# ComputationalRobotics/cuADMM

Measured on AMD Instinct MI355X. Metric: ADMM iters/sec, 10k x 32-blk synthetic per GPU (+ PSD-proj TFLOP/s in roofline), higher is better.
Workload: dtype f64

## Files before the change

### cuadmm_amd/_lib.py

```python
import ctypes as C
import os

from . import build as _build

_HERE = os.path.dirname(os.path.abspath(__file__))
LIB_PATH = os.path.join(_HERE, "lib", "libcuadmm_amd.so")

c_int_p = C.POINTER(C.c_int)
c_double_p = C.POINTER(C.c_double)
ALLREDUCE_FN = C.CFUNCTYPE(C.c_int, C.c_void_p, C.c_void_p, C.c_size_t, C.c_void_p)


class ProblemView(C.Structure):
    _fields_ = [("vec_len", C.c_int), ("con_num", C.c_int), ("mat_num", C.c_int),
                ("At_nnz", C.c_int), ("b_nnz", C.c_int), ("C_nnz", C.c_int),
                ("At_csc_col_ptrs", c_int_p), ("At_csc_row_ids", c_int_p), ("At_csc_vals", c_double_p),
                ("b_indices", c_int_p), ("b_vals", c_double_p), ("C_indices", c_int_p), ("C_vals", c_double_p),
                ("blk_vals", c_int_p)]


PROTOTYPES = {
    "cuadmm_last_error": (C.c_char_p, []),
    "cuadmm_version": (C.c_char_p, []),
    "cuadmm_device_count": (C.c_int, []),
# ... 27 lines not shown
    "cuadmm_get_shard": (C.c_int, [C.c_void_p, C.POINTER(C.c_int64), C.POINTER(C.c_int64), c_int_p, c_int_p]),
    "cuadmm_aat_factor_arrays": (C.c_int, [C.c_void_p] + [C.POINTER(C.c_void_p)] * 4),
    "cuadmm_aat_forest": (C.c_int, [C.c_void_p, c_int_p, c_int_p, C.POINTER(C.c_void_p), C.POINTER(C.c_void_p)]),
    "cuadmm_mex_call": (C.c_int, [C.c_int, C.c_int, C.c_double,
                                   C.c_size_t, C.c_size_t, C.c_void_p, C.c_void_p, C.c_void_p,
                                   C.c_size_t, C.c_void_p, C.c_void_p, C.c_void_p,
                                   C.c_size_t, C.c_void_p, C.c_void_p, C.c_void_p,
                                   C.c_size_t, C.c_void_p,
                                   C.c_size_t, C.c_void_p, C.c_size_t, C.c_void_p, C.c_size_t, C.c_void_p,
                                   C.c_double, C.c_int, C.c_void_p, C.POINTER(C.c_void_p)]),
    "cuadmm_mex_result_dims": (C.c_int, [C.c_void_p, c_int_p, c_int_p, c_int_p, C.POINTER(C.c_double)]),
    "cuadmm_mex_result_XyS": (C.c_int, [C.c_void_p, C.c_void_p, C.c_void_p, C.c_void_p]),
    "cuadmm_mex_result_info": (C.c_int, [C.c_void_p, C.c_int, C.c_void_p]),
    "cuadmm_mex_result_free": (None, [C.c_void_p]),
    "cuadmm_get_psd_steps": (C.c_int, [C.c_void_p, C.c_void_p, C.c_int]),
    "cuadmm_sign_sched_simulate_hint": (C.c_int, [C.c_void_p, C.c_int, C.c_int, C.c_int, c_double_p, c_int_p]),
    "cuadmm_sign_sched_simulate": (C.c_int, [C.c_void_p, C.c_int, C.c_int, c_double_p]),
    "cuadmm_op_psd_project_ex": (C.c_int, [C.c_void_p, C.c_void_p, C.c_void_p, C.c_int, C.c_int, C.c_void_p, C.c_void_p]),
    "cuadmm_op_psd_project_steps": (C.c_int, [C.c_void_p, C.c_void_p, C.c_void_p, C.c_int, C.c_void_p, C.c_void_p]),
    "cuadmm_get_info_iter_num": (C.c_int, [C.c_void_p]),
    "cuadmm_get_info_array": (C.c_int, [C.c_void_p, C.c_int, C.c_void_p, C.c_int]),
    "cuadmm_get_total_time": (C.c_double, [C.c_void_p]),
    "cuadmm_get_state": (C.c_int, [C.c_void_p, C.c_void_p]),
    "cuadmm_get_profile": (C.c_int, [C.c_void_p, C.c_void_p]),
    "cuadmm_reset_profile": (C.c_int, [C.c_void_p]),
    "cuadmm_get_counters": (C.c_int, [C.c_void_p, C.c_void_p]),
    "cuadmm_get_group_info": (C.c_int, [C.c_void_p, C.c_void_p]),
    "cuadmm_get_tail_info": (C.c_int, [C.c_void_p, C.c_void_p]),
    "cuadmm_update_A": (C.c_int, [C.c_void_p, C.c_void_p, C.c_int, C.c_int, C.c_double]),
    "cuadmm_get_update_info": (C.c_int, [C.c_void_p, C.c_void_p]),
# ... 118 lines not shown
```

### cuadmm_amd/csrc/engine.hip

```cpp
#include <hip/hip_runtime.h>

#include <algorithm>
#include <chrono>
#include <cmath>
#include <cstdlib>
#include <cstring>
#include <dlfcn.h>
#include <iostream>
#include <numeric>

#include "device_util.h"
#include "psd_plan.h"
#include "tail_solve.h"
#include "lead_solve.h"
#include "vec_kernels.h"
#include "duo_group.h"
#include "accel.h"
#include "infeas.h"

using namespace cuadmm;

namespace {

double wall_s() { return std::chrono::duration<double>(std::chrono::steady_clock::now().time_since_epoch()).count(); }
// ... 501 lines not shown
      fz.outX = mode == 0 ? out_w : nullptr;
      fz.outS = out_w + m + 2;
    }
    if (closed.active) {
      fz.rec = closed.rec.p; fz.cl_out = closed.cl_out.p; fz.y_out = y_d.p;
      fz.iter0 = (int)(closed.iters_done & 0x3fffffff);
      closed.iters_done += iters > 1 ? iters : 1;
      fz.partials2 = closed.partials2.p;
      fz.isig = 1 / sig; fz.bscale = bscale;
      if (closed.out_dirty) {
        if ((rc = launch_closed_gather_out(closed.rec.p, plan.fused_blocks(), out_d.p, out_d.p + (size_t)m + 2, closed.cl_out.p, st))) return rc;
        closed.out_dirty = false;
      }
    }
    if (iters > 1) {
      fz.iters = iters; fz.pstride = bt.pstride; fz.partials = bt.p1.p; fz.partials2 = bt.p2.p;
      prof_begin(K_PSD);
      rc = plan.project(Xb.p, Xproj.p, st, &fz);
      prof_end(K_PSD, 68.0 * (double)L * iters);
      if (rc) return rc;
      prof_begin(K_POST);
      double* dst = (!dev_scalars && bt.h_dev) ? bt.h_dev : bt.scal_d.p;
      rc = launch_reduce_quads_batch(bt.p1.p, bt.p2.p, plan.fused_blocks(), bt.pstride, iters, dst, st);
      prof_end(K_POST, 0.0);
      if (rc) return rc;
      if (dev_scalars && (rc = comm_allreduce(bt.scal_d.p, 4 * (size_t)iters))) return rc;
      if (dst == bt.scal_d.p) CUADMM_HIP_TRY(hipMemcpyAsync(bt.h.p, bt.scal_d.p, sizeof(double) * 4 * (size_t)iters, hipMemcpyDeviceToHost, st));
      bt.launches++; bt.iters += iters;
      return CUADMM_OK;
    }
    prof_begin(K_PSD);
// ... 2112 lines not shown

int cuadmm_get_profile(const cuadmm_solver* s, double out[3 * CUADMM_NUM_KCLASS]) {
  if (!s || !out) { set_error("get_profile: null"); return CUADMM_ERR_INVALID; }
  for (int k = 0; k < K_NUM; ++k) { out[3 * k] = s->prof_count[k]; out[3 * k + 1] = s->prof_ms[k]; out[3 * k + 2] = s->prof_bytes[k]; }
  return CUADMM_OK;
}
int cuadmm_get_psd_steps(cuadmm_solver* s, int* out, int cap) {
  if (!s || !out) { set_error("get_psd_steps: null"); return CUADMM_ERR_INVALID; }
  if (!s->steps_d.p && s->psd_steps && s->initialised && s->blk_local.empty()) return 0;
  if (!s->steps_d.p) { set_error("get_psd_steps: set option psd_steps=1 before init"); return CUADMM_ERR_INVALID; }
  const int n = (int)std::min<size_t>(s->steps_d.n, (size_t)std::max(cap, 0));
  CUADMM_HIP_TRY(hipStreamSynchronize(s->st));
  { int rc2 = staged_d2h(out, s->steps_d.p, sizeof(int) * (size_t)n, s->st); if (rc2) return rc2; }
  return n;
}
int cuadmm_get_counters(const cuadmm_solver* s, double o[8]) {
  if (!s || !o) { set_error("get_counters: null"); return CUADMM_ERR_INVALID; }
  o[0] = (double)s->bt.launches; o[1] = (double)s->bt.iters; o[2] = (double)s->bt.rollbacks; o[3] = (double)cuadmm_host_pool_threads();
  o[4] = s->fuse ? 1 : 0; o[5] = s->closed.active ? 1 : 0; o[6] = s->dev_solve ? (s->lead.tops ? 3 : 1) : (s->lead.hybrid ? 2 : 0); o[7] = (double)s->tail.k;
  return CUADMM_OK;
}
int cuadmm_get_accel_info(const cuadmm_solver* s, double o[8]) {
  if (!s || !o) { set_error("get_accel_info: null"); return CUADMM_ERR_INVALID; }
  o[0] = (double)s->aa.mem; o[1] = (double)s->aa.taken; o[2] = (double)s->aa.accepted; o[3] = (double)s->aa.rejected; o[4] = (double)s->aa.restarts;
  o[5] = (double)s->aa.cols; o[6] = s->profile ? s->aa.ms : 0.0; o[7] = (double)(s->aa.ring_dF.n + s->aa.ring_dG.n) * sizeof(double);
  return CUADMM_OK;
}
int cuadmm_accel_solve_ls(const double* gram, const double* rhs, int cols, double reg, double* gamma_out) {
  return accel_solve_ls(gram, rhs, cols, reg, gamma_out);
}
// ... 408 lines not shown
```

### cuadmm_amd/csrc/psd_fuse.h

```cpp
#pragma once

namespace cuadmm {

struct SignFuse {
  const int* rp; const int* ci; const double* av;
  const double* y; const double* C;
  double* X; double* Rd1; double* S;
  double* partials;
  double sig, inv_sig, tau_sig;
  int mode;
  const struct LcDesc* lc; const int* lc_row; const int* lc_nzptr; const int* lc_e; const double* lc_v;
  double* outX; double* outS;
  double* y_out;
  double* partials2;
  double isig, bscale;
  int iters;
  long long pstride;
  const struct ClosedRec* rec;
  double* cl_out;
  int iter0;
  int full;
};
struct LcDesc { int x, y, z, w; };
constexpr int kFuseRowsMax = 64;
constexpr int kClosedMaxRows = 8;

struct alignas(64) ClosedRec {
  int nk, nnz, nrounds, maxlen;
  unsigned char nzp[16];
  int rows[kClosedMaxRows];
  unsigned nzt[kFuseRowsMax];
  unsigned char rk[kFuseRowsMax];
// ... 13 lines not shown
```

### cuadmm_amd/csrc/psd_kernels.hip

```cpp
#include <hip/hip_runtime.h>

#include <algorithm>
#include <cstdio>
#include <cstdlib>
#include <string>
#include <vector>

#include "device_util.h"
#include "eig_large.h"
#include "psd_device.h"
#include "psd_plan.h"
#include "psd_small_reg.h"
#include "psd_sign_lds.h"
#include "psd_sign_wave.h"
#include "psd_sign_closed.h"

namespace cuadmm {

struct PsdArgs {
  const double* in;
  double* out;
  double* Wout;
  int* info;
  const int* ids;
// ... 102 lines not shown
  if (m >= count) return;
  const PsdDesc d = a.desc[first + m];
  const int id = d.id;
  const long long off = d.off;
  psd_sign_wave_body<NT, FUSED, !(NT == 1 && OCC == 8)>(a.in + off, a.out + off, d.n, a.info, swt_smem, a.steps ? a.steps + id : nullptr,
                                a.hint ? a.hint + id : nullptr, a.dbg ? a.dbg + 10 * (long long)m : nullptr, fz, off, d.slot, id);
}

template <int NT, int OCC, bool FULL>
__global__ __launch_bounds__(64) __attribute__((amdgpu_waves_per_eu(OCC, OCC))) void psd_sign_closed_kernel(ClosedArgs a) {
  extern __shared__ double swt_smem[];
  const int m = (int)blockIdx.x;
  if (m >= a.count) return;
  const PsdDesc d = a.desc[a.first + m];
  SwcKArg ka = (SwcKArg)__builtin_amdgcn_kernarg_segment_ptr();
  psd_sign_closed_body<NT, false, FULL>(a, d.n, swt_smem, a.steps ? a.steps + d.id : nullptr, a.hint ? a.hint + d.id : nullptr, nullptr, d.off, d.slot, 0, d.pad[0], 0, ka);
}

__host__ __device__ constexpr int closed_cu_ctl_ints(int nb_max) { return (nb_max + 2 + 3) & ~3; }
static_assert(sizeof(PsdDesc) == 32, "the LDS descriptor cache copies a descriptor as two 16-byte words");

template <int NT, int WAVES, int OCC, bool FULL, bool DBG>
__global__ __launch_bounds__(64 * WAVES) __attribute__((amdgpu_waves_per_eu(OCC, OCC))) void psd_sign_closed_cu_kernel(ClosedArgs a) {
  extern __shared__ double swt_smem[];
  constexpr int TILE = SignWaveT<NT>::NP * SignWaveT<NT>::LD;
  int* ctl = reinterpret_cast<int*>(swt_smem + (size_t)WAVES * TILE);
  const int g = (int)blockIdx.x, G = (int)gridDim.x;
  const int nb = (a.count - g + G - 1) / G;
  for (int i = (int)threadIdx.x; i < nb + 1; i += 64 * WAVES) ctl[i] = 0;
  sl_v4i32* dcache = reinterpret_cast<sl_v4i32*>(ctl + closed_cu_ctl_ints((a.count + G - 1) / G));
  if (a.dcache)
    for (int i = (int)threadIdx.x; i < nb; i += 64 * WAVES) {
      const sl_v4i32* src = reinterpret_cast<const sl_v4i32*>(a.desc + a.first + g + i * G);
      dcache[2 * i] = src[0];
      dcache[2 * i + 1] = src[1];
    }
  __syncthreads();
  const int ntask = nb * a.iters;
  const long long clk0 = (DBG && a.dbg) ? (long long)__builtin_readcyclecounter() : 0, rt0 = (DBG && a.dbg) ? (long long)__builtin_amdgcn_s_memrealtime() : 0;
  using KArgC = __attribute__((address_space(4))) const char;
  KArgC* ka = (KArgC*)__builtin_amdgcn_kernarg_segment_ptr();
#pragma unroll 1
  for (;;) {
    const long long tk0 = (DBG && a.dbg) ? (long long)__builtin_readcyclecounter() : 0;
    int t = 0;
    if (lane_id() == 0) t = atomicAdd(&ctl[0], 1);
    t = __builtin_amdgcn_readfirstlane(t);
    if (t >= ntask) break;
    const int it = t / nb, j = t - it * nb;
    if (it > 0) {
      while (__hip_atomic_load(ctl + 1 + j, __ATOMIC_RELAXED, __HIP_MEMORY_SCOPE_WORKGROUP) < it) __builtin_amdgcn_s_sleep(8);
    }
    __builtin_amdgcn_fence(__ATOMIC_ACQUIRE, "workgroup");
    const long long tk1 = (DBG && a.dbg) ? (long long)__builtin_readcyclecounter() : 0;
#if defined(__HIP_DEVICE_COMPILE__)
    asm volatile("" : "+s"(ka));
    const ClosedArgs al = *reinterpret_cast<__attribute__((address_space(4))) const ClosedArgs*>(ka);
#else
    const ClosedArgs al = a;
    (void)ka;
#endif
    PsdDesc d;
    if (al.dcache) {
      const sl_v4i32 q0 = dcache[2 * j], q1 = dcache[2 * j + 1];
      d.off = (long long)(((unsigned long long)(unsigned)__builtin_amdgcn_readfirstlane(q0[1]) << 32) | (unsigned)__builtin_amdgcn_readfirstlane(q0[0]));
      d.n = __builtin_amdgcn_readfirstlane(q0[2]); d.id = __builtin_amdgcn_readfirstlane(q0[3]); d.slot = __builtin_amdgcn_readfirstlane(q1[0]);
      d.pad[0] = __builtin_amdgcn_readfirstlane(q1[1]);
    } else {
      d = al.desc[al.first + g + j * G];
    }
    int toff = ((int)threadIdx.x >> 6) * TILE;
#if defined(__HIP_DEVICE_COMPILE__)
    asm volatile("" : "+v"(toff));
#endif
    double* tile = swt_smem + toff;
    const long long tk2 = (DBG && al.dbg) ? (long long)__builtin_readcyclecounter() : 0;
    psd_sign_closed_body<NT, true, FULL, DBG>(al, d.n, tile, al.steps ? al.steps + d.id : nullptr, al.hint ? al.hint + d.id : nullptr,
                             (DBG && al.dbg) ? al.dbg + 16 * (long long)(g + j * G) : nullptr, d.off, d.slot, (long long)it * al.pstride, d.pad[0], it, ka);
    const long long tk3 = (DBG && al.dbg) ? (long long)__builtin_readcyclecounter() : 0;
    __builtin_amdgcn_fence(__ATOMIC_RELEASE, "workgroup");
    if (lane_id() == 0) __hip_atomic_store(ctl + 1 + j, it + 1, __ATOMIC_RELAXED, __HIP_MEMORY_SCOPE_WORKGROUP);
    if (DBG && al.dbg && lane_id() == 0) {
      long long* q = al.dbg + 16 * (long long)(g + j * G);
      q[10] = tk1 - tk0; q[11] = tk2 - tk1; q[12] = tk3 - tk2; q[13] = (long long)__builtin_readcyclecounter() - tk3;
    }
  }
  if (DBG && a.dbg && threadIdx.x == 0) {
    long long* q = a.dbg + 16 * (long long)g;
    q[14] = (long long)__builtin_readcyclecounter() - clk0; q[15] = (long long)__builtin_amdgcn_s_memrealtime() - rt0;
  }
}

template <void (*KERN)(ClosedArgs)>
static int launch_closed_cu(dim3 grid, dim3 block, size_t lds, hipStream_t st, const ClosedArgs& ca) {
  static LdsCapOnce once;
  CUADMM_HIP_TRY(once(reinterpret_cast<const void*>(KERN)));
  hipLaunchKernelGGL(KERN, grid, block, lds, st, ca);
  return CUADMM_OK;
}

template <int NT, int OCC>
static int launch_sign_wave(const PsdArgs& a, int first, int count, hipStream_t st, const SignFuse* fz = nullptr) {
  if (count <= 0) return CUADMM_OK;
  if (fz && fz->rec) {
    ClosedArgs ca{};
    ca.desc = a.desc; ca.steps = a.steps; ca.hint = a.hint; ca.fail = a.info; ca.dbg = a.dbg;
    ca.X = fz->X; ca.S = fz->S; ca.Rd1 = fz->Rd1; ca.C = fz->C; ca.rec = fz->rec; ca.cl_out = fz->cl_out; ca.y_out = fz->y_out;
    ca.outS = fz->outS; ca.outX = fz->outX; ca.partials = fz->partials; ca.partials2 = fz->partials2;
    ca.sig = fz->sig; ca.inv_sig = fz->inv_sig; ca.tau_sig = fz->tau_sig; ca.isig = fz->isig; ca.bscale = fz->bscale;
    ca.iter0 = fz->iter0;
    ca.pstride = fz->pstride; ca.mode = fz->mode; ca.iters = fz->iters > 1 ? fz->iters : 1; ca.first = first; ca.count = count;
    if (fz->iters > 1) {
      constexpr int WAVES = 4 * OCC > 16 ? 16 : 4 * OCC, WG_PER_CU = 4 * OCC / WAVES;
      static int n_cu_of[64] = {0};
      int dev = 0;
      CUADMM_HIP_TRY(hipGetDevice(&dev));
      int& n_cu = n_cu_of[dev & 63];
      if (n_cu == 0) {
        int v = 0;
        CUADMM_HIP_TRY(hipDeviceGetAttribute(&v, hipDeviceAttributeMultiprocessorCount, dev));
        n_cu = v > 0 ? v : 256;
      }
      const int grid = std::min(count, n_cu * WG_PER_CU);
      const size_t nb_max = ((size_t)count + grid - 1) / grid;
      size_t lds = WAVES * SignWaveT<NT>::LDS_BYTES + sizeof(int) * (size_t)closed_cu_ctl_ints((int)nb_max);
      ca.dcache = lds + sizeof(PsdDesc) * nb_max <= kMaxLdsBytes;
      if (ca.dcache) lds += sizeof(PsdDesc) * nb_max;
      if (lds > kMaxLdsBytes) { set_error("psd: %d blocks per workgroup do not fit the batched launch", (int)nb_max); return CUADMM_ERR_INVALID; }
      constexpr bool HAS_DBG = NT == 2 && OCC == 4;
      const dim3 gr(grid), bl(64 * WAVES);
      int rc;
      if (HAS_DBG && ca.dbg) rc = fz->full ? launch_closed_cu<psd_sign_closed_cu_kernel<NT, WAVES, OCC, true, HAS_DBG>>(gr, bl, lds, st, ca)
                                           : launch_closed_cu<psd_sign_closed_cu_kernel<NT, WAVES, OCC, false, HAS_DBG>>(gr, bl, lds, st, ca);
      else rc = fz->full ? launch_closed_cu<psd_sign_closed_cu_kernel<NT, WAVES, OCC, true, false>>(gr, bl, lds, st, ca)
                         : launch_closed_cu<psd_sign_closed_cu_kernel<NT, WAVES, OCC, false, false>>(gr, bl, lds, st, ca);
      if (rc) return rc;
    } else if (fz->full) {
      hipLaunchKernelGGL((psd_sign_closed_kernel<NT, OCC, true>), dim3(count), dim3(64), SignWaveT<NT>::LDS_BYTES, st, ca);
// ... 497 lines not shown
```

### cuadmm_amd/csrc/psd_options.h

```cpp
#pragma once
#include <cstdlib>
#include <cstring>
#include <string>

namespace cuadmm {

struct PsdOptions {
  int n16_sign = 1;
  int n32_sign = 1;
  int mid = 0;
  int wave4_min = 1024;
  int w32_occ = 4;
  int cu_occ = 4;
  int lds_triple = 1;
  int sign_min = 65;
  int overlap = 1;
  int lg_tile = 0;
  int lg_pad32 = 1;
  int lg_decide = 0;
  int lg_merge = 1;
  int lg_fuse = 1;
  int lg_cluster_wgs = 224;
  int lg_cluster = 1;
  int sign_maxsteps = 0;
  int sign_sync = 1;
  int sign_ws_mb = 8192;
  int debug = 0;

  static PsdOptions from_env() {
    PsdOptions o;
    static const struct { const char* env; const char* key; } tab[] = {
        {"CUADMM_PSD_DEBUG", "psd_debug"},           {"CUADMM_PSD_WAVE4_MIN", "psd_wave4_min"}, {"CUADMM_PSD_SIGN_MIN", "psd_sign_min"},
        {"CUADMM_PSD_W32_OCC", "psd_w32_occ"},       {"CUADMM_PSD_CU_OCC", "psd_cu_occ"},       {"CUADMM_PSD_OVERLAP", "psd_overlap"},
        {"CUADMM_PSD_N16", "psd_n16"},               {"CUADMM_PSD_N32", "psd_n32"},             {"CUADMM_PSD_MID", "psd_mid"},
        {"CUADMM_PSD_LG_CLUSTER", "psd_lg_cluster"}, {"CUADMM_PSD_LDS_TRIPLE", "psd_lds_triple"}, {"CUADMM_PSD_LG_MERGE", "psd_lg_merge"},
        {"CUADMM_PSD_LG_FUSE", "psd_lg_fuse"},       {"CUADMM_PSD_LG_CLUSTER_WGS", "psd_lg_cluster_wgs"}};
    for (const auto& t : tab)
      if (const char* e = getenv(t.env)) {
        int v;
        if (!strcmp(e, "eig")) v = strcmp(t.key, "psd_mid") ? 0 : 1;
        else if (!strcmp(e, "lds")) v = 2;
        else v = atoi(e);
        o.set(t.key, v);
      }
    return o;
  }
  bool set(const std::string& k, double value) {
    const int v = (int)value;
    if (k == "psd_n16") n16_sign = v;
    else if (k == "psd_n32") n32_sign = v;
    else if (k == "psd_mid") mid = v;
    else if (k == "psd_wave4_min") wave4_min = v;
    else if (k == "psd_w32_occ") w32_occ = v == 3 ? 3 : 4;
    else if (k == "psd_cu_occ") cu_occ = v == 3 ? 3 : 4;
    else if (k == "psd_lds_triple") lds_triple = v;
    else if (k == "psd_sign_min") sign_min = v < 65 ? 65 : v;
    else if (k == "psd_overlap") overlap = v;
    else if (k == "psd_lg_tile") lg_tile = v;
    else if (k == "psd_lg_pad32") lg_pad32 = v;
    else if (k == "psd_lg_decide") lg_decide = v;
    else if (k == "psd_lg_cluster") lg_cluster = v;
    else if (k == "psd_lg_merge") lg_merge = v;
    else if (k == "psd_lg_fuse") lg_fuse = v;
    else if (k == "psd_lg_cluster_wgs") lg_cluster_wgs = v < 8 ? 8 : (v > 960 ? 960 : v);
    else if (k == "psd_sign_maxsteps") sign_maxsteps = v;
    else if (k == "psd_sign_sync") sign_sync = v;
    else if (k == "psd_sign_ws_mb") sign_ws_mb = v < 1 ? 1 : v;
    else if (k == "psd_debug") debug = v < 0 ? 0 : v;
    else return false;
// ... 6 lines not shown
```

### cuadmm_amd/csrc/psd_sign_closed.h

```cpp
#pragma once
#include <hip/hip_runtime.h>

#include "psd_sign_wave.h"

namespace cuadmm {

template <int LD>
__device__ __forceinline__ int swc_sym(int row, int col) { return row <= col ? row * LD + col : col * LD + row; }
template <int LD, int NP>
__device__ __forceinline__ int swc_low(int r, int c) { return r == c ? r * LD + NP : c * LD + r; }

template <int NT>
__device__ __forceinline__ void swc_frags(const double* __restrict__ M, int r16, int kk, double (&f)[4 * NT][NT]) {
  constexpr int LD = SignWaveT<NT>::LD;
#pragma unroll
  for (int s = 0; s < 4 * NT; ++s)
#pragma unroll
    for (int x = 0; x < NT; ++x) {
      const int b = s / 4, row = 4 * s + kk, col = 16 * x + r16;
      if (x > b) f[s][x] = M[row * LD + col];
      else if (x < b) f[s][x] = M[col * LD + row];
      else f[s][x] = M[swc_sym<LD>(row, col)];
    }
}
// ... 78 lines not shown
template <int NT> __device__ const SwcTab<NT> g_swc_tab = SwcTab<NT>();

struct ClosedArgs {
  const PsdDesc* desc;
  int* steps; int* hint; int* fail;
  long long* dbg;
  double* X; double* S; double* Rd1; const double* C;
  const ClosedRec* rec;
  double* cl_out; double* y_out; double* outS; double* outX;
  double* partials; double* partials2;
  double sig, inv_sig, tau_sig, isig, bscale;
  long long pstride;
  int mode, iters, first, count;
  int iter0;
  int dcache;
};

using SwcKArg = __attribute__((address_space(4))) const char*;
template <bool RELOAD>
__device__ __forceinline__ ClosedArgs swc_args(const ClosedArgs& fz, SwcKArg& ka) {
#if defined(__HIP_DEVICE_COMPILE__)
  if (RELOAD) {
    asm volatile("" : "+s"(ka));
    return *reinterpret_cast<__attribute__((address_space(4))) const ClosedArgs*>(ka);
  }
#endif
  return fz;
}

#define CUADMM_SWC_STAMP(k) \
  if (dbg) { asm volatile("s_waitcnt vmcnt(0) lgkmcnt(0)" ::: "memory"); if (lane == 0) dbg[k] = (long long)__builtin_readcyclecounter() - c0; }

template <int NT, bool TASK_LOOP = false, bool FULL = false, bool DBG = false>
__device__ __forceinline__ void psd_sign_closed_body(const ClosedArgs& fz, int n_arg, double* S, int* steps_out, int* hint, long long* dbg_arg,
                                                     long long off, int slot, long long poff, int hdr, int it_local, SwcKArg ka) {
  long long* const dbg = DBG ? dbg_arg : nullptr;
  using Cfg = SignWaveT<NT>;
  constexpr int LD = Cfg::LD, NP = Cfg::NP, U = Cfg::U, NSLOT = Cfg::NSLOT;
  constexpr int NB = (NSLOT + U - 1) / U;
  const int n = FULL ? NP : n_arg;
  int lane_p = lane_id();
#if defined(__HIP_DEVICE_COMPILE__)
  if (TASK_LOOP) asm volatile("" : "+v"(lane_p));
  __builtin_assume(lane_p >= 0 && lane_p < 64);
#endif
  const int lane = lane_p;
  const int r16 = lane & 15, kk = lane >> 4;
  const int len = n * (n + 1) / 2;
  const int ksteps = FULL ? 4 * NT : ((n + 3) >> 2);
  const long long c0 = dbg ? (long long)__builtin_readcyclecounter() : 0;
  const bool upd = fz.mode == 0;
  const ClosedRec* __restrict__ rec = fz.rec + slot;
  const unsigned* __restrict__ tabl = g_swc_tab<NT>.v + lane;
  const double* __restrict__ Xl = fz.X + off + lane;
  const double* __restrict__ Cl = fz.C + off + lane;
  auto at = [&](unsigned byte_off) -> double& { return *reinterpret_cast<double*>(reinterpret_cast<char*>(S) + byte_off); };

  const int nk = closed_hdr_nk(hdr), nnz = closed_hdr_nnz(hdr), nrounds = closed_hdr_nrounds(hdr);
  const int l8 = lane & 7;
  const bool mine = lane < nk;
  const double nzv = rec->v[lane];
  const unsigned nzt = rec->nzt[lane];
  const int nzrk = rec->rk[lane];
  const int row = rec->rows[l8];
  const double dk = rec->D[l8], bk = rec->b[l8];
  const double ax_old = fz.cl_out[16 * (long long)slot + l8], as_old = fz.cl_out[16 * (long long)slot + 8 + l8];
  double lrow[kClosedMaxRows], lcol[kClosedMaxRows];
#pragma unroll
  for (int q = 0; q < kClosedMaxRows; ++q) {
    lrow[q] = rec->L[l8 * kClosedMaxRows + q];
    lcol[q] = rec->L[q * kClosedMaxRows + l8];
  }
  unsigned tb[U];
  double xv[U], cv[U];
#pragma unroll
  for (int u = 0; u < U; ++u) { tb[u] = tabl[64 * u]; xv[u] = Xl[64 * u]; cv[u] = Cl[64 * u]; }
  {
    sl_v2f64* S2 = reinterpret_cast<sl_v2f64*>(S);
    double zero = 0.0;
#if defined(__HIP_DEVICE_COMPILE__)
    if (TASK_LOOP) asm volatile("" : "+v"(zero));
#endif
#pragma unroll 1
    for (int i = lane; i < NP * LD / 2; i += 64) S2[i] = sl_v2f64{zero, zero};
    wave_fence();
  }
  double yk = 0.0;
  if (nk > 0) {
    const double rp = __dadd_rn(-ax_old, bk);
    double x = mine ? __dadd_rn(-as_old, __dmul_rn(fz.isig, rp)) : 0.0;
#pragma unroll
// ... 39 lines not shown
      if (ok_) {
        at(lo) = r1;
        if (!upd) fz.Rd1[off + e_] = r1;
        ss += xb * xb;
        at(up) = (tb[u] & 1u) ? xb : xb * kSqrt2Inv;
      }
    }
  }
  CUADMM_SWC_STAMP(6);
  const double nrm = sqrt(wave_sum(ss));
  const double scale = nrm > 0.0 ? 1.0 / nrm : (nrm == 0.0 ? 0.0 : nrm);
  wave_fence();
  double f[4 * NT][NT];
  SignSchedPlain sched;
  if (hint) {
    int h = __builtin_amdgcn_readfirstlane(*hint);
    if (h > 1 && (((unsigned)fz.iter0 + (unsigned)it_local + (unsigned)slot) & 15u) == 15u) --h;
    if (h > 0) sched.lift0 = h;
  }
  bool last = false;
  const long long c1 = dbg ? (long long)__builtin_readcyclecounter() : 0;
  while (!last) {
    swc_frags<NT>(S, r16, kk, f);
    if (sched.steps == 0) {
#pragma unroll
      for (int s = 0; s < 4 * NT; ++s)
#pragma unroll
        for (int x = 0; x < NT; ++x) f[s][x] *= scale;
    }
    wave_fence();
    sl_v4f64 y[NT][NT];
// ... 48 lines not shown
    }
    double alpha, beta;
    sched.coefs(mu, alpha, beta);
#pragma unroll
    for (int i = 0; i < NT; ++i)
#pragma unroll
      for (int j = i; j < NT; ++j)
#pragma unroll
        for (int r = 0; r < 4; ++r) z[i][j][r] = fma(alpha, z[i][j][r], beta * f[4 * i + r][j]);
    wave_fence();
    swc_store_upper<NT>(S, r16, kk, z);
    wave_fence();
  }
  if (steps_out && lane == 0) *steps_out = sched.steps;
  if (hint && lane == 0) *hint = sched.lifts;
  const long long c2 = dbg ? (long long)__builtin_readcyclecounter() : 0;
  int lane_e = lane;
#if defined(__HIP_DEVICE_COMPILE__)
  asm volatile("" : "+v"(lane_e));
#endif
  const unsigned* __restrict__ tabl_e = g_swc_tab<NT>.v + lane_e;
  const ClosedArgs fe = swc_args<true>(fz, ka);
  const ClosedRec* __restrict__ rec_e = fe.rec + slot;
  const double* __restrict__ Xl_e = fe.X + off + lane_e;
  const double* __restrict__ Cl_e = fe.C + off + lane_e;
  const int l8e = lane_e & 7;
  const bool mine_e = lane_e < nk;
#pragma unroll
  for (int u = 0; u < U; ++u) { tb[u] = tabl_e[64 * u]; xv[u] = Xl_e[64 * u]; }
  swc_frags<NT>(S, r16, kk, f);
// ... 77 lines not shown
#pragma unroll
    for (int u = 0; u < U; ++u) {
      const int e_ = base + 64 * u + lane_e;
      const bool ok_ = (FULL && base + 64 * u + 63 < Cfg::MAXLEN) || e_ < len;
      const unsigned up = tb[u] & 0xfff8u, lo = tb[u] >> 16;
      const double pm = at(up), r1 = at(lo);
      bad |= ok_ && !(fabs(pm) <= 1.7976931348623157e308);
      const double xp = (tb[u] & 1u) ? pm : pm * kSqrt2;
      const double x = xv[u];
      const double xdiff = xp - x;
      const double sv = fw.inv_sig * xdiff - r1;
      double xn = x;
      double rd = 0.0;
      if (upd) { rd = r1 + sv; xn = x + fw.tau_sig * rd; }
      if (ok_) {
        Sg[base + 64 * u] = sv;
        if (upd) {
          Xg[base + 64 * u] = xn;
          s_rd += rd * rd;
          s_cx += cv[u] * xn;
        }
        at(up) = sv - cv[u];
        at(lo) = xn;
      }
      if ((u % 3) == 2) swc_sched_split();
    }
  }
  CUADMM_SWC_STAMP(9);
  {
    wave_fence();
    const double ps = nzv_e * at(nzt_e & 0xfff8u);
    const double px = nzv_e * at(nzt_e >> 16);
    const int maxlen = closed_hdr_maxlen(hdr);
    double as = 0.0, ax = 0.0;
    for (int t = 0; t < maxlen; ++t) {
      const int src = (kb + t) & 63;
      const double vs = __shfl(ps, src, 64), vx = __shfl(px, src, 64);
      if (mine_e && kb + t < ke) { as += vs; ax += vx; }
    }
    if (mine_e) {
      fw.outS[row_e] = as;
      fw.cl_out[16 * (long long)slot + 8 + lane_e] = as;
      if (upd) { fw.outX[row_e] = ax; fw.cl_out[16 * (long long)slot + lane_e] = ax; }
    }
    if (upd) {
      const double ro = nrmA_e * (bk_e - ax) * fw.bscale;
      double pr = mine_e ? ro * ro : 0.0;
      pr = wave_sum(pr);
      const double pby = pby_sum;
      s_rd = wave_sum(s_rd);
      s_cx = wave_sum(s_cx);
      if (lane_e == 0) {
        fw.partials2[poff + 2 * (long long)slot] = pr; fw.partials2[poff + 2 * (long long)slot + 1] = pby;
        fw.partials[poff + 2 * (long long)slot] = s_rd; fw.partials[poff + 2 * (long long)slot + 1] = s_cx;
      }
    }
  }
  if (bad && fw.fail) atomicAdd(fw.fail, 1);
  if (dbg && lane == 0) {
// ... 8 lines not shown
```

### cuadmm_amd/solver.py

```python
import ctypes as C

import numpy as np

from . import _lib
from ._lib import check

_INFO = {"pobj": 0, "dobj": 1, "errRp": 2, "errRd": 3, "relgap": 4, "sig": 5, "bscale": 6, "Cscale": 7}


def _i32(a):
    return np.ascontiguousarray(a, dtype=np.int32)


def _f64(a):
    return np.ascontiguousarray(a, dtype=np.float64)


def _p(a):
    return None if a is None else a.ctypes.data_as(C.c_void_p)


class Problem:

    def __init__(self, vec_len, con_num, blk_vals, At_csc_col_ptrs, At_csc_row_ids, At_csc_vals,
# ... 257 lines not shown
        return dict(zip(keys, o.tolist()))

    def profile(self):
        o = np.zeros(24)
        check(self._lib.cuadmm_get_profile(self._h, _p(o)))
        names = ["aty_xb", "psd_project", "post_proj", "spmv_A", "copies", "host", "allreduce", "tail_solve"]
        return {n: dict(launches=o[3 * i], ms=o[3 * i + 1], bytes_per_launch=o[3 * i + 2]) for i, n in enumerate(names)}

    def psd_steps(self):
        b, e, kb, ke = self.shard()
        out = np.zeros(max(ke - kb, 1), np.int32)
        n = self._lib.cuadmm_get_psd_steps(self._h, _p(out), out.size)
        check(min(n, 0))
        return out[:n]

    def reset_profile(self):
        check(self._lib.cuadmm_reset_profile(self._h))
```

### include/cuadmm_amd.h

```cpp
#ifndef CUADMM_AMD_H
#define CUADMM_AMD_H

#include <stddef.h>
#include <stdint.h>

#ifdef __cplusplus
extern "C" {
#endif

#define CUADMM_OK 0
#define CUADMM_ERR_INVALID (-1)
#define CUADMM_ERR_NO_DEVICE (-2)
#define CUADMM_ERR_IO (-3)
#define CUADMM_ERR_FACTOR (-4)
#define CUADMM_ERR_EIG (-5)
#define CUADMM_ERR_COMM (-6)
#define CUADMM_ERR_ALLOC (-7)
#define CUADMM_ERR_INTERNAL (-8)

const char* cuadmm_last_error(void);
const char* cuadmm_version(void);
int cuadmm_device_count(void);

typedef struct cuadmm_solver cuadmm_solver;
// ... 54 lines not shown
#define CUADMM_INFO_ERRRP 2
#define CUADMM_INFO_ERRRD 3
#define CUADMM_INFO_RELGAP 4
#define CUADMM_INFO_SIG 5
#define CUADMM_INFO_BSCALE 6
#define CUADMM_INFO_CSCALE 7
int cuadmm_get_info_iter_num(const cuadmm_solver* s);
int cuadmm_get_info_array(const cuadmm_solver* s, int which, double* out, int cap);
double cuadmm_get_total_time(const cuadmm_solver* s);
int cuadmm_get_state(const cuadmm_solver* s, double out12[12]);

#define CUADMM_NUM_KCLASS 8
int cuadmm_get_profile(const cuadmm_solver* s, double out[3 * CUADMM_NUM_KCLASS]);
int cuadmm_reset_profile(cuadmm_solver* s);
int cuadmm_get_psd_steps(cuadmm_solver* s, int* out, int cap);
int cuadmm_get_counters(const cuadmm_solver* s, double out8[8]);
int cuadmm_get_tail_info(const cuadmm_solver* s, double out[6]);
int cuadmm_get_accel_info(const cuadmm_solver* s, double out8[8]);
int cuadmm_accel_solve_ls(const double* gram, const double* rhs, int cols, double reg, double* gamma_out);
int cuadmm_get_status(const cuadmm_solver* s, double out8[8]);
int cuadmm_get_certificate(cuadmm_solver* s, double* y_out, double* X_out);
int cuadmm_infeas_decide(const double stats[8], double tol, int* verdict, double* radius);
int cuadmm_get_group_info(const cuadmm_solver* s, double out4[4]);

typedef struct cuadmm_problem cuadmm_problem;
typedef struct {
  int vec_len, con_num, mat_num;
  int At_nnz, b_nnz, C_nnz;
  const int* At_csc_col_ptrs;
  const int* At_csc_row_ids;
// ... 128 lines not shown
```

Measured before the change: 5058.

## Run consecutive ADMM iterations per block in closed PSD task loop with register carry

The persistent closed-form PSD kernel now processes a run of consecutive iterations (default 2) for the same block within one task, rather than one iteration per task. Per-block state (X, C, table entries, record values, hint, ax/as) is carried in registers between iterations, which avoids global reloads and skips the intermediate S stores that later iterations overwrite. The aim is to cut global memory traffic and atomic task-scheduling overhead. In exchange, the pipeline across blocks gets coarser, which can worsen load balance, and register pressure rises. An optional workgroup cap and a debug accessor for the PSD hints are also added.

```diff
diff --git a/cuadmm_amd/_lib.py b/cuadmm_amd/_lib.py
--- a/cuadmm_amd/_lib.py
+++ b/cuadmm_amd/_lib.py
@@ -65,6 +65,7 @@
     "cuadmm_mex_result_info": (C.c_int, [C.c_void_p, C.c_int, C.c_void_p]),
     "cuadmm_mex_result_free": (None, [C.c_void_p]),
     "cuadmm_get_psd_steps": (C.c_int, [C.c_void_p, C.c_void_p, C.c_int]),
+    "cuadmm_get_psd_hints": (C.c_int, [C.c_void_p, C.c_void_p, C.c_int]),
     "cuadmm_sign_sched_simulate_hint": (C.c_int, [C.c_void_p, C.c_int, C.c_int, C.c_int, c_double_p, c_int_p]),
     "cuadmm_sign_sched_simulate": (C.c_int, [C.c_void_p, C.c_int, C.c_int, c_double_p]),
     "cuadmm_op_psd_project_ex": (C.c_int, [C.c_void_p, C.c_void_p, C.c_void_p, C.c_int, C.c_int, C.c_void_p, C.c_void_p]),
diff --git a/cuadmm_amd/csrc/engine.hip b/cuadmm_amd/csrc/engine.hip
--- a/cuadmm_amd/csrc/engine.hip
+++ b/cuadmm_amd/csrc/engine.hip
@@ -539,7 +539,7 @@
       }
     }
     if (iters > 1) {
-      fz.iters = iters; fz.pstride = bt.pstride; fz.partials = bt.p1.p; fz.partials2 = bt.p2.p;
+      fz.iters = iters; fz.run = plan.opt.cu_run; fz.wgs = plan.opt.cu_wgs; fz.pstride = bt.pstride; fz.partials = bt.p1.p; fz.partials2 = bt.p2.p;
       prof_begin(K_PSD);
       rc = plan.project(Xb.p, Xproj.p, st, &fz);
       prof_end(K_PSD, 68.0 * (double)L * iters);
@@ -2682,6 +2682,14 @@
   { int rc2 = staged_d2h(out, s->steps_d.p, sizeof(int) * (size_t)n, s->st); if (rc2) return rc2; }
   return n;
 }
+int cuadmm_get_psd_hints(cuadmm_solver* s, int* out, int cap) {
+  if (!s || !out) { set_error("get_psd_hints: null"); return CUADMM_ERR_INVALID; }
+  if (!s->hint_d.p) return 0;
+  const int n = (int)std::min<size_t>(s->hint_d.n, (size_t)std::max(cap, 0));
+  CUADMM_HIP_TRY(hipStreamSynchronize(s->st));
+  { int rc2 = staged_d2h(out, s->hint_d.p, sizeof(int) * (size_t)n, s->st); if (rc2) return rc2; }
+  return n;
+}
 int cuadmm_get_counters(const cuadmm_solver* s, double o[8]) {
   if (!s || !o) { set_error("get_counters: null"); return CUADMM_ERR_INVALID; }
   o[0] = (double)s->bt.launches; o[1] = (double)s->bt.iters; o[2] = (double)s->bt.rollbacks; o[3] = (double)cuadmm_host_pool_threads();
diff --git a/cuadmm_amd/csrc/psd_fuse.h b/cuadmm_amd/csrc/psd_fuse.h
--- a/cuadmm_amd/csrc/psd_fuse.h
+++ b/cuadmm_amd/csrc/psd_fuse.h
@@ -16,6 +16,8 @@
   double isig, bscale;
   int iters;
   long long pstride;
+  int wgs;
+  int run;
   const struct ClosedRec* rec;
   double* cl_out;
   int iter0;
diff --git a/cuadmm_amd/csrc/psd_kernels.hip b/cuadmm_amd/csrc/psd_kernels.hip
--- a/cuadmm_amd/csrc/psd_kernels.hip
+++ b/cuadmm_amd/csrc/psd_kernels.hip
@@ -140,7 +140,10 @@
   if (m >= a.count) return;
   const PsdDesc d = a.desc[a.first + m];
   SwcKArg ka = (SwcKArg)__builtin_amdgcn_kernarg_segment_ptr();
-  psd_sign_closed_body<NT, false, FULL>(a, d.n, swt_smem, a.steps ? a.steps + d.id : nullptr, a.hint ? a.hint + d.id : nullptr, nullptr, d.off, d.slot, 0, d.pad[0], 0, ka);
+  SwcCarry<NT> cy;
+  swc_head<NT>(cy, a, a.hint ? a.hint + d.id : nullptr, d.off, d.slot);
+  psd_sign_closed_body<NT, false, FULL>(a, d.n, swt_smem, a.steps ? a.steps + d.id : nullptr, a.hint ? a.hint + d.id : nullptr, nullptr, d.off, d.slot, 0, d.pad[0], 0, ka,
+                                        cy, false, true);
 }
 
 __host__ __device__ constexpr int closed_cu_ctl_ints(int nb_max) { return (nb_max + 2 + 3) & ~3; }
@@ -162,7 +165,7 @@
       dcache[2 * i + 1] = src[1];
     }
   __syncthreads();
-  const int ntask = nb * a.iters;
+  const int ntask = nb * ((a.iters + (a.run > 1 ? a.run : 1) - 1) / (a.run > 1 ? a.run : 1));
   const long long clk0 = (DBG && a.dbg) ? (long long)__builtin_readcyclecounter() : 0, rt0 = (DBG && a.dbg) ? (long long)__builtin_amdgcn_s_memrealtime() : 0;
   using KArgC = __attribute__((address_space(4))) const char;
   KArgC* ka = (KArgC*)__builtin_amdgcn_kernarg_segment_ptr();
@@ -173,41 +176,60 @@
     if (lane_id() == 0) t = atomicAdd(&ctl[0], 1);
     t = __builtin_amdgcn_readfirstlane(t);
     if (t >= ntask) break;
-    const int it = t / nb, j = t - it * nb;
-    if (it > 0) {
-      while (__hip_atomic_load(ctl + 1 + j, __ATOMIC_RELAXED, __HIP_MEMORY_SCOPE_WORKGROUP) < it) __builtin_amdgcn_s_sleep(8);
+    const int rn = t / nb, j = t - rn * nb;
+    if (rn > 0) {
+      while (__hip_atomic_load(ctl + 1 + j, __ATOMIC_RELAXED, __HIP_MEMORY_SCOPE_WORKGROUP) < rn) __builtin_amdgcn_s_sleep(8);
     }
     __builtin_amdgcn_fence(__ATOMIC_ACQUIRE, "workgroup");
     const long long tk1 = (DBG && a.dbg) ? (long long)__builtin_readcyclecounter() : 0;
+    long long tk2 = 0, tk3 = 0;
 #if defined(__HIP_DEVICE_COMPILE__)
     asm volatile("" : "+s"(ka));
-    const ClosedArgs al = *reinterpret_cast<__attribute__((address_space(4))) const ClosedArgs*>(ka);
+    const ClosedArgs ah = *reinterpret_cast<__attribute__((address_space(4))) const ClosedArgs*>(ka);
 #else
-    const ClosedArgs al = a;
+    const ClosedArgs ah = a;
     (void)ka;
 #endif
     PsdDesc d;
-    if (al.dcache) {
+    if (ah.dcache) {
       const sl_v4i32 q0 = dcache[2 * j], q1 = dcache[2 * j + 1];
       d.off = (long long)(((unsigned long long)(unsigned)__builtin_amdgcn_readfirstlane(q0[1]) << 32) | (unsigned)__builtin_amdgcn_readfirstlane(q0[0]));
       d.n = __builtin_amdgcn_readfirstlane(q0[2]); d.id = __builtin_amdgcn_readfirstlane(q0[3]); d.slot = __builtin_amdgcn_readfirstlane(q1[0]);
       d.pad[0] = __builtin_amdgcn_readfirstlane(q1[1]);
     } else {
-      d = al.desc[al.first + g + j * G];
-    }
-    int toff = ((int)threadIdx.x >> 6) * TILE;
+      d = ah.desc[ah.first + g + j * G];
+    }
+    SwcCarry<NT> cy;
+    swc_head<NT>(cy, ah, ah.hint ? ah.hint + d.id : nullptr, d.off, d.slot);
+    if (DBG) tk2 = ah.dbg ? (long long)__builtin_readcyclecounter() : 0;
+    const int R = ah.run > 1 ? ah.run : 1;
+    int it = rn * R;
+    const int it_end = (it + R < ah.iters ? it + R : ah.iters) - 1;
+#pragma unroll 1
+    for (;;) {
 #if defined(__HIP_DEVICE_COMPILE__)
-    asm volatile("" : "+v"(toff));
+      asm volatile("" : "+s"(ka));
+      const ClosedArgs al = *reinterpret_cast<__attribute__((address_space(4))) const ClosedArgs*>(ka);
+#else
+      const ClosedArgs al = a;
 #endif
-    double* tile = swt_smem + toff;
-    const long long tk2 = (DBG && al.dbg) ? (long long)__builtin_readcyclecounter() : 0;
-    psd_sign_closed_body<NT, true, FULL, DBG>(al, d.n, tile, al.steps ? al.steps + d.id : nullptr, al.hint ? al.hint + d.id : nullptr,
-                             (DBG && al.dbg) ? al.dbg + 16 * (long long)(g + j * G) : nullptr, d.off, d.slot, (long long)it * al.pstride, d.pad[0], it, ka);
-    const long long tk3 = (DBG && al.dbg) ? (long long)__builtin_readcyclecounter() : 0;
+      int toff = ((int)threadIdx.x >> 6) * TILE;
+#if defined(__HIP_DEVICE_COMPILE__)
+      asm volatile("" : "+v"(toff));
+#endif
+      double* tile = swt_smem + toff;
+      const bool more = it < it_end;
+      psd_sign_closed_body<NT, true, FULL, DBG>(al, d.n, tile, al.steps ? al.steps + d.id : nullptr, al.hint ? al.hint + d.id : nullptr,
+                               (DBG && al.dbg) ? al.dbg + 16 * (long long)(g + j * G) : nullptr, d.off, d.slot, (long long)it * al.pstride, d.pad[0], it, ka,
+                               cy, more, it + 1 >= al.iters);
+      if (!more) break;
+      ++it;
+    }
+    if (DBG) tk3 = a.dbg ? (long long)__builtin_readcyclecounter() : 0;
     __builtin_amdgcn_fence(__ATOMIC_RELEASE, "workgroup");
-    if (lane_id() == 0) __hip_atomic_store(ctl + 1 + j, it + 1, __ATOMIC_RELAXED, __HIP_MEMORY_SCOPE_WORKGROUP);
-    if (DBG && al.dbg && lane_id() == 0) {
-      long long* q = al.dbg + 16 * (long long)(g + j * G);
+    if (lane_id() == 0) __hip_atomic_store(ctl + 1 + j, rn + 1, __ATOMIC_RELAXED, __HIP_MEMORY_SCOPE_WORKGROUP);
+    if (DBG && a.dbg && lane_id() == 0) {
+      long long* q = a.dbg + 16 * (long long)(g + j * G);
       q[10] = tk1 - tk0; q[11] = tk2 - tk1; q[12] = tk3 - tk2; q[13] = (long long)__builtin_readcyclecounter() - tk3;
     }
   }
@@ -235,7 +257,7 @@
     ca.outS = fz->outS; ca.outX = fz->outX; ca.partials = fz->partials; ca.partials2 = fz->partials2;
     ca.sig = fz->sig; ca.inv_sig = fz->inv_sig; ca.tau_sig = fz->tau_sig; ca.isig = fz->isig; ca.bscale = fz->bscale;
     ca.iter0 = fz->iter0;
-    ca.pstride = fz->pstride; ca.mode = fz->mode; ca.iters = fz->iters > 1 ? fz->iters : 1; ca.first = first; ca.count = count;
+    ca.pstride = fz->pstride; ca.mode = fz->mode; ca.iters = fz->iters > 1 ? fz->iters : 1; ca.run = fz->run; ca.first = first; ca.count = count;
     if (fz->iters > 1) {
       constexpr int WAVES = 4 * OCC > 16 ? 16 : 4 * OCC, WG_PER_CU = 4 * OCC / WAVES;
       static int n_cu_of[64] = {0};
@@ -247,7 +269,7 @@
         CUADMM_HIP_TRY(hipDeviceGetAttribute(&v, hipDeviceAttributeMultiprocessorCount, dev));
         n_cu = v > 0 ? v : 256;
       }
-      const int grid = std::min(count, n_cu * WG_PER_CU);
+      const int grid = std::min(std::min(count, n_cu * WG_PER_CU), fz->wgs > 0 ? fz->wgs : count);
       const size_t nb_max = ((size_t)count + grid - 1) / grid;
       size_t lds = WAVES * SignWaveT<NT>::LDS_BYTES + sizeof(int) * (size_t)closed_cu_ctl_ints((int)nb_max);
       ca.dcache = lds + sizeof(PsdDesc) * nb_max <= kMaxLdsBytes;
diff --git a/cuadmm_amd/csrc/psd_options.h b/cuadmm_amd/csrc/psd_options.h
--- a/cuadmm_amd/csrc/psd_options.h
+++ b/cuadmm_amd/csrc/psd_options.h
@@ -12,6 +12,8 @@
   int wave4_min = 1024;
   int w32_occ = 4;
   int cu_occ = 4;
+  int cu_run = 2;
+  int cu_wgs = 0;
   int lds_triple = 1;
   int sign_min = 65;
   int overlap = 1;
@@ -34,7 +36,8 @@
         {"CUADMM_PSD_W32_OCC", "psd_w32_occ"},       {"CUADMM_PSD_CU_OCC", "psd_cu_occ"},       {"CUADMM_PSD_OVERLAP", "psd_overlap"},
         {"CUADMM_PSD_N16", "psd_n16"},               {"CUADMM_PSD_N32", "psd_n32"},             {"CUADMM_PSD_MID", "psd_mid"},
         {"CUADMM_PSD_LG_CLUSTER", "psd_lg_cluster"}, {"CUADMM_PSD_LDS_TRIPLE", "psd_lds_triple"}, {"CUADMM_PSD_LG_MERGE", "psd_lg_merge"},
-        {"CUADMM_PSD_LG_FUSE", "psd_lg_fuse"},       {"CUADMM_PSD_LG_CLUSTER_WGS", "psd_lg_cluster_wgs"}};
+        {"CUADMM_PSD_LG_FUSE", "psd_lg_fuse"},       {"CUADMM_PSD_LG_CLUSTER_WGS", "psd_lg_cluster_wgs"},
+        {"CUADMM_PSD_CU_RUN", "psd_cu_run"}};
     for (const auto& t : tab)
       if (const char* e = getenv(t.env)) {
         int v;
@@ -53,6 +56,8 @@
     else if (k == "psd_wave4_min") wave4_min = v;
     else if (k == "psd_w32_occ") w32_occ = v == 3 ? 3 : 4;
     else if (k == "psd_cu_occ") cu_occ = v == 3 ? 3 : 4;
+    else if (k == "psd_cu_run") cu_run = v < 1 ? 1 : (v > 256 ? 256 : v);
+    else if (k == "psd_cu_wgs") cu_wgs = v < 0 ? 0 : v;
     else if (k == "psd_lds_triple") lds_triple = v;
     else if (k == "psd_sign_min") sign_min = v < 65 ? 65 : v;
     else if (k == "psd_overlap") overlap = v;
diff --git a/cuadmm_amd/csrc/psd_sign_closed.h b/cuadmm_amd/csrc/psd_sign_closed.h
--- a/cuadmm_amd/csrc/psd_sign_closed.h
+++ b/cuadmm_amd/csrc/psd_sign_closed.h
@@ -116,6 +116,7 @@
   int mode, iters, first, count;
   int iter0;
   int dcache;
+  int run;
 };
 
 using SwcKArg = __attribute__((address_space(4))) const char*;
@@ -130,12 +131,47 @@
   return fz;
 }
 
+template <int NT>
+struct SwcCarry {
+  static constexpr int U = SignWaveT<NT>::U;
+  double x[U], c[U];
+  unsigned tb[U];
+  double nzv; unsigned nzt;
+  int row; double bk;
+  double ax, as;
+  int hint;
+};
+template <int NT>
+__device__ __forceinline__ void swc_head(SwcCarry<NT>& cy, const ClosedArgs& fz, const int* hint, long long off, int slot) {
+  constexpr int U = SignWaveT<NT>::U;
+  int lane = lane_id();
+#if defined(__HIP_DEVICE_COMPILE__)
+  asm volatile("" : "+v"(lane));
+  __builtin_assume(lane >= 0 && lane < 64);
+#endif
+  const int l8 = lane & 7;
+  const ClosedRec* __restrict__ rec = fz.rec + slot;
+  const unsigned* __restrict__ tabl = g_swc_tab<NT>.v + lane;
+  const double* __restrict__ Xl = fz.X + off + lane;
+  const double* __restrict__ Cl = fz.C + off + lane;
+  cy.nzv = rec->v[lane];
+  cy.nzt = rec->nzt[lane];
+  cy.row = rec->rows[l8];
+  cy.bk = rec->b[l8];
+  cy.ax = fz.cl_out[16 * (long long)slot + l8];
+  cy.as = fz.cl_out[16 * (long long)slot + 8 + l8];
+#pragma unroll
+  for (int u = 0; u < U; ++u) { cy.tb[u] = tabl[64 * u]; cy.x[u] = Xl[64 * u]; cy.c[u] = Cl[64 * u]; }
+  cy.hint = hint ? __builtin_amdgcn_readfirstlane(*hint) : 0;
+}
+
 #define CUADMM_SWC_STAMP(k) \
   if (dbg) { asm volatile("s_waitcnt vmcnt(0) lgkmcnt(0)" ::: "memory"); if (lane == 0) dbg[k] = (long long)__builtin_readcyclecounter() - c0; }
 
 template <int NT, bool TASK_LOOP = false, bool FULL = false, bool DBG = false>
 __device__ __forceinline__ void psd_sign_closed_body(const ClosedArgs& fz, int n_arg, double* S, int* steps_out, int* hint, long long* dbg_arg,
-                                                     long long off, int slot, long long poff, int hdr, int it_local, SwcKArg ka) {
+                                                     long long off, int slot, long long poff, int hdr, int it_local, SwcKArg ka,
+                                                     SwcCarry<NT>& cy, bool more, bool store_s) {
   long long* const dbg = DBG ? dbg_arg : nullptr;
   using Cfg = SignWaveT<NT>;
   constexpr int LD = Cfg::LD, NP = Cfg::NP, U = Cfg::U, NSLOT = Cfg::NSLOT;
@@ -152,21 +188,22 @@
   const int ksteps = FULL ? 4 * NT : ((n + 3) >> 2);
   const long long c0 = dbg ? (long long)__builtin_readcyclecounter() : 0;
   const bool upd = fz.mode == 0;
-  const ClosedRec* __restrict__ rec = fz.rec + slot;
   const unsigned* __restrict__ tabl = g_swc_tab<NT>.v + lane;
   const double* __restrict__ Xl = fz.X + off + lane;
   const double* __restrict__ Cl = fz.C + off + lane;
   auto at = [&](unsigned byte_off) -> double& { return *reinterpret_cast<double*>(reinterpret_cast<char*>(S) + byte_off); };
 
   const int nk = closed_hdr_nk(hdr), nnz = closed_hdr_nnz(hdr), nrounds = closed_hdr_nrounds(hdr);
+  const bool mine = lane < nk;
+  const double nzv = cy.nzv;
+  const unsigned nzt = cy.nzt;
+  const int row = cy.row;
+  const double bk = cy.bk;
+  const double ax_old = cy.ax, as_old = cy.as;
+  const ClosedRec* __restrict__ rec = fz.rec + slot;
   const int l8 = lane & 7;
-  const bool mine = lane < nk;
-  const double nzv = rec->v[lane];
-  const unsigned nzt = rec->nzt[lane];
   const int nzrk = rec->rk[lane];
-  const int row = rec->rows[l8];
-  const double dk = rec->D[l8], bk = rec->b[l8];
-  const double ax_old = fz.cl_out[16 * (long long)slot + l8], as_old = fz.cl_out[16 * (long long)slot + 8 + l8];
+  const double dk = rec->D[l8];
   double lrow[kClosedMaxRows], lcol[kClosedMaxRows];
 #pragma unroll
   for (int q = 0; q < kClosedMaxRows; ++q) {
@@ -176,7 +213,7 @@
   unsigned tb[U];
   double xv[U], cv[U];
 #pragma unroll
-  for (int u = 0; u < U; ++u) { tb[u] = tabl[64 * u]; xv[u] = Xl[64 * u]; cv[u] = Cl[64 * u]; }
+  for (int u = 0; u < U; ++u) { tb[u] = cy.tb[u]; xv[u] = cy.x[u]; cv[u] = cy.c[u]; }
   {
     sl_v2f64* S2 = reinterpret_cast<sl_v2f64*>(S);
     double zero = 0.0;
@@ -246,7 +283,7 @@
   double f[4 * NT][NT];
   SignSchedPlain sched;
   if (hint) {
-    int h = __builtin_amdgcn_readfirstlane(*hint);
+    int h = cy.hint;
     if (h > 1 && (((unsigned)fz.iter0 + (unsigned)it_local + (unsigned)slot) & 15u) == 15u) --h;
     if (h > 0) sched.lift0 = h;
   }
@@ -325,6 +362,7 @@
   }
   if (steps_out && lane == 0) *steps_out = sched.steps;
   if (hint && lane == 0) *hint = sched.lifts;
+  cy.hint = sched.lifts;
   const long long c2 = dbg ? (long long)__builtin_readcyclecounter() : 0;
   int lane_e = lane;
 #if defined(__HIP_DEVICE_COMPILE__)
@@ -432,7 +470,7 @@
       double rd = 0.0;
       if (upd) { rd = r1 + sv; xn = x + fw.tau_sig * rd; }
       if (ok_) {
-        Sg[base + 64 * u] = sv;
+        if (store_s) Sg[base + 64 * u] = sv;
         if (upd) {
           Xg[base + 64 * u] = xn;
           s_rd += rd * rd;
@@ -441,10 +479,18 @@
         at(up) = sv - cv[u];
         at(lo) = xn;
       }
+      if (NB == 1) xv[u] = xn;
       if ((u % 3) == 2) swc_sched_split();
     }
   }
   CUADMM_SWC_STAMP(9);
+  if (NB > 1 && more) {
+#pragma unroll
+    for (int u = 0; u < U; ++u) { tb[u] = tabl_e[64 * u]; xv[u] = Xg[64 * u]; cv[u] = Cl_e[64 * u]; }
+  }
+#pragma unroll
+  for (int u = 0; u < U; ++u) { cy.tb[u] = tb[u]; cy.x[u] = xv[u]; cy.c[u] = cv[u]; }
+  cy.nzv = nzv_e; cy.nzt = nzt_e; cy.row = row_e; cy.bk = bk_e;
   {
     wave_fence();
     const double ps = nzv_e * at(nzt_e & 0xfff8u);
@@ -461,6 +507,7 @@
       fw.cl_out[16 * (long long)slot + 8 + lane_e] = as;
       if (upd) { fw.outX[row_e] = ax; fw.cl_out[16 * (long long)slot + lane_e] = ax; }
     }
+    cy.ax = ax; cy.as = as;
     if (upd) {
       const double ro = nrmA_e * (bk_e - ax) * fw.bscale;
       double pr = mine_e ? ro * ro : 0.0;
diff --git a/cuadmm_amd/solver.py b/cuadmm_amd/solver.py
--- a/cuadmm_amd/solver.py
+++ b/cuadmm_amd/solver.py
@@ -295,5 +295,12 @@
         check(min(n, 0))
         return out[:n]
 
+    def psd_hints(self):
+        b, e, kb, ke = self.shard()
+        out = np.zeros(max(ke - kb, 1), np.int32)
+        n = self._lib.cuadmm_get_psd_hints(self._h, _p(out), out.size)
+        check(min(n, 0))
+        return out[:n]
+
     def reset_profile(self):
         check(self._lib.cuadmm_reset_profile(self._h))
diff --git a/include/cuadmm_amd.h b/include/cuadmm_amd.h
--- a/include/cuadmm_amd.h
+++ b/include/cuadmm_amd.h
@@ -92,6 +92,7 @@
 int cuadmm_get_profile(const cuadmm_solver* s, double out[3 * CUADMM_NUM_KCLASS]);
 int cuadmm_reset_profile(cuadmm_solver* s);
 int cuadmm_get_psd_steps(cuadmm_solver* s, int* out, int cap);
+int cuadmm_get_psd_hints(cuadmm_solver* s, int* out, int cap);
 int cuadmm_get_counters(const cuadmm_solver* s, double out8[8]);
 int cuadmm_get_tail_info(const cuadmm_solver* s, double out[6]);
 int cuadmm_get_accel_info(const cuadmm_solver* s, double out8[8]);
```

Result: no change. 5061, median of 3 (+0.1%).
